# llm-d/llm-d-inference-scheduler

Measured on AMD Instinct MI355X. Metric: routed req/s + p50 EPP latency; P/D goodput (tok/s under TTFT SLO) Llama-3-8B, higher is better.
Workload: dtype bf16; 1 GPU; model=llama-3-8b, global_batch=256, seq_len=2048, parallelism=dp1, mode=mono, prompt_len=1024, kv_cache_dtype=bfloat16, warmup_steps_run=32, errors=0

## Files before the change

csrc/hip/hip_common.h:

```cpp
#pragma once
#include <hip/hip_runtime.h>
#include <hip/hip_bf16.h>
#include <cstdint>
#include <type_traits>

#define WAVE 64

typedef __attribute__((ext_vector_type(8))) short short8;
typedef __attribute__((ext_vector_type(4))) short short4v;
typedef __attribute__((ext_vector_type(4))) float float4v;
typedef __attribute__((ext_vector_type(2))) float float2v;

__device__ __forceinline__ float bf16_to_f32(short u) {
  union { float f; uint32_t i; } c;
  c.i = ((uint32_t)(uint16_t)u) << 16;
  return c.f;
}

__device__ __forceinline__ short f32_to_bf16(float f) {
  union { float f; uint32_t i; } c;
  c.f = f;
  uint32_t lsb = (c.i >> 16) & 1;
  uint32_t rounded = c.i + 0x7FFF + lsb;
  return (short)(uint16_t)(rounded >> 16);
}

typedef __attribute__((ext_vector_type(8))) unsigned char uchar8;

__device__ __forceinline__ void load_kv8(const short* p, float* f) {
  short8 v = *(const short8*)p;
#pragma unroll
  for (int j = 0; j < 8; ++j) f[j] = bf16_to_f32(v[j]);
}

__device__ __forceinline__ void load_kv8(const unsigned char* p, float* f) {
  const uint32_t* w = (const uint32_t*)p;
  uint32_t a = w[0], b = w[1];
  f[0] = __builtin_amdgcn_cvt_f32_fp8(a, 0);
  f[1] = __builtin_amdgcn_cvt_f32_fp8(a, 1);
  f[2] = __builtin_amdgcn_cvt_f32_fp8(a, 2);
  f[3] = __builtin_amdgcn_cvt_f32_fp8(a, 3);
  f[4] = __builtin_amdgcn_cvt_f32_fp8(b, 0);
  f[5] = __builtin_amdgcn_cvt_f32_fp8(b, 1);
  f[6] = __builtin_amdgcn_cvt_f32_fp8(b, 2);
  f[7] = __builtin_amdgcn_cvt_f32_fp8(b, 3);
}

__device__ __forceinline__ void load_kv2(const short* p, float& a, float& b) {
  const int32_t pair = *(const int32_t*)p;
  a = bf16_to_f32((short)(pair & 0xFFFF));
  b = bf16_to_f32((short)((pair >> 16) & 0xFFFF));
}

__device__ __forceinline__ void load_kv2(const unsigned char* p, float& a,
                                         float& b) {
  const uint32_t pair = *(const uint16_t*)p;
  a = __builtin_amdgcn_cvt_f32_fp8(pair, 0);
// ... 102 lines not shown
```

csrc/hip/launchers.h:

```cpp
#pragma once
#include <hip/hip_runtime.h>
#include <cstdint>


hipError_t lds_hash_prompts(const int32_t* tokens, const int64_t* offsets,
                            int n_requests, int block_tokens, int max_blocks,
                            uint64_t seed0, uint64_t* out, int32_t* counts,
                            hipStream_t stream);
hipError_t lds_table_update(uint64_t* keys, unsigned long long* masks,
                            uint32_t cap_mask, const uint64_t* hashes,
                            int64_t n, int endpoint, int is_remove,
                            unsigned int* dropped, hipStream_t stream);
hipError_t lds_match_longest(const uint64_t* keys,
                             const unsigned long long* masks,
                             uint32_t cap_mask, const uint64_t* hashes,
                             const int32_t* counts, int n_requests,
                             int max_blocks, int n_endpoints, int32_t* out,
                             hipStream_t stream);


hipError_t lds_rmsnorm(const void* x, void* residual, const void* w, void* y,
                       int64_t n_rows, int H, float eps, hipStream_t stream);
hipError_t lds_rope(void* q, void* k, const float* cos_sin,
                    const int32_t* positions, int n_tokens, int n_q_heads,
                    int n_kv_heads, int head_dim, hipStream_t stream);
hipError_t lds_silu_mul(const void* gate_up, void* y, int64_t T, int I,
                        hipStream_t stream);


hipError_t lds_reshape_and_cache(const void* k_new, const void* v_new,
                                 void* k_cache, void* v_cache,
                                 const int64_t* slots, int n_tokens, int kvh,
                                 int bs, int d, int kv_fp8,
                                 const float* k_inv_scale,
                                 const float* v_inv_scale,
                                 hipStream_t stream);
hipError_t lds_gather_blocks(const void* pool, void* staging,
                             const int32_t* block_ids, int n_sel, int n_layers,
                             int64_t n_blocks, int64_t block_bytes,
                             int is_scatter, hipStream_t stream);
hipError_t lds_copy_blocks_peer(const void* src_pool, void* dst_pool,
                                const int32_t* src_ids, const int32_t* dst_ids,
                                int n_sel, int n_layers, int64_t src_nb,
                                int64_t dst_nb, int64_t block_bytes,
                                hipStream_t stream);


constexpr int FLASH_GLDS_BT_CAP = 1024;

struct AttnArgs {
  const void* q;
  const void* k_cache;
  const void* v_cache;
  const int32_t* block_tables;
  void* out;
  const float* k_scale;
  const float* v_scale;
  int n_q_heads, kvh, bs, head_dim, max_blocks;
  int kv_fp8;
  float scale;
// ... 56 lines not shown
```

csrc/hip/norm_rope_act.hip:

```cpp
#include "hip_common.h"
#include "launchers.h"

namespace {

constexpr int RMSNORM_WAVES = 4;

template <bool RESIDUAL>
__global__ void rmsnorm_kernel(const short* __restrict__ x,
                               short* __restrict__ residual,
                               const short* __restrict__ w,
                               short* __restrict__ y, int H, float eps) {
  constexpr int CACHE_CHUNKS = 8;
  __shared__ float red[16];
  const int64_t row = blockIdx.x;
  const int tid = threadIdx.x;
  const int nthreads = blockDim.x;
  const short8* x8 = (const short8*)(x + row * H);
  short8* r8 = RESIDUAL ? (short8*)(residual + row * H) : nullptr;
  const short8* w8 = (const short8*)w;
  short8* y8 = (short8*)(y + row * H);
  const int nchunks = H / 8;

  float vals[CACHE_CHUNKS][8];
  float ss = 0.f;
// ... 25 lines not shown
  ci = 0;
  for (int c = tid; c < nchunks; c += nthreads, ++ci) {
    float f[8];
    if (ci < CACHE_CHUNKS) {
#pragma unroll
      for (int j = 0; j < 8; ++j) f[j] = vals[ci][j];
    } else {
      short8 v = RESIDUAL ? r8[c] : x8[c];
#pragma unroll
      for (int j = 0; j < 8; ++j) f[j] = bf16_to_f32(v[j]);
    }
    short8 wv = w8[c];
    short8 o;
#pragma unroll
    for (int j = 0; j < 8; ++j) o[j] = f32_to_bf16(f[j] * inv * bf16_to_f32(wv[j]));
    y8[c] = o;
  }
}

__global__ void rope_kernel(short* __restrict__ q, short* __restrict__ k,
                            const float* __restrict__ cos_sin,
                            const int32_t* __restrict__ positions, int n_tokens,
                            int n_q_heads, int n_kv_heads, int D) {
  const int t = blockIdx.x;
  const int head = blockIdx.y;
  const int half = D / 2;
  const int lane = threadIdx.x;
  if (t >= n_tokens || lane >= half) return;
  short* base = (head < n_q_heads)
                    ? q + ((int64_t)t * n_q_heads + head) * D
                    : k + ((int64_t)t * n_kv_heads + (head - n_q_heads)) * D;
  const float* cs = cos_sin + ((int64_t)positions[t] * half + lane) * 2;
  const float c = cs[0], s = cs[1];
  float x1 = bf16_to_f32(base[lane]);
  float x2 = bf16_to_f32(base[lane + half]);
  base[lane] = f32_to_bf16(x1 * c - x2 * s);
  base[lane + half] = f32_to_bf16(x2 * c + x1 * s);
}

__global__ void silu_mul_kernel(const short* __restrict__ gate_up,
                                short* __restrict__ y, int64_t T, int I) {
  const int nchunks = I / 8;
  const int64_t total = T * nchunks;
  for (int64_t i = (int64_t)blockIdx.x * blockDim.x + threadIdx.x; i < total;
       i += (int64_t)gridDim.x * blockDim.x) {
    int64_t row = i / nchunks;
    int c = (int)(i % nchunks);
    const short8* g8 = (const short8*)(gate_up + row * 2 * I);
    const short8* u8 = (const short8*)(gate_up + row * 2 * I + I);
    short8 g = g8[c], u = u8[c];
    short8 o;
#pragma unroll
    for (int j = 0; j < 8; ++j) {
      float gf = bf16_to_f32(g[j]);
      float uf = bf16_to_f32(u[j]);
      float sig = 1.f / (1.f + __expf(-gf));
      o[j] = f32_to_bf16(gf * sig * uf);
    }
    ((short8*)(y + row * I))[c] = o;
  }
}

}

hipError_t lds_rmsnorm(const void* x, void* residual, const void* w, void* y,
                       int64_t n_rows, int H, float eps, hipStream_t stream) {
  if (n_rows == 0) return hipSuccess;
  dim3 grid((uint32_t)n_rows), block(RMSNORM_WAVES * WAVE);
  if (residual) {
    hipLaunchKernelGGL(rmsnorm_kernel<true>, grid, block, 0, stream,
// ... 37 lines not shown
```

csrc/hip/ops.hip:

```cpp
#include <torch/extension.h>
#include <ATen/hip/HIPContext.h>
#include <ATen/hip/impl/HIPStreamMasqueradingAsCUDA.h>

#include <hip/hip_runtime.h>

#include <climits>

#include "launchers.h"

#define CHECK_HIP(expr)                                                    \
  do {                                                                     \
    hipError_t err__ = (expr);                                             \
    TORCH_CHECK(err__ == hipSuccess, "HIP error: ", hipGetErrorString(err__)); \
  } while (0)

#define CHECK_GPU(t) TORCH_CHECK((t).is_cuda() && (t).is_contiguous(), #t " must be contiguous on GPU")

namespace {

int kv_fp8_flag(const torch::Tensor& cache) {
  if (cache.scalar_type() == at::kFloat8_e4m3fn) return 1;
  TORCH_CHECK(cache.scalar_type() == at::kBFloat16,
              "KV cache must be bf16 or fp8_e4m3fn");
  return 0;
// ... 204 lines not shown
  auto y = torch::empty(sizes, gate_up.options());
  CHECK_HIP(lds_silu_mul(gate_up.data_ptr(), y.data_ptr(), T, I,
                         cur_stream()));
  return y;
}

void reshape_and_cache(torch::Tensor k_new, torch::Tensor v_new,
                       torch::Tensor k_cache, torch::Tensor v_cache,
                       torch::Tensor slots,
                       c10::optional<torch::Tensor> k_inv_scale,
                       c10::optional<torch::Tensor> v_inv_scale) {
  check_tensor(k_new, "k_new", k_new, "k_new", at::kBFloat16,
               {ANY, ANY, ANY});
  const int64_t T = k_new.size(0), KVH = k_new.size(1), D = k_new.size(2);
  TORCH_CHECK(D % 8 == 0, "head dim k_new.size(2) must be a multiple of 8, "
              "got ", D);
  check_int(KVH * (D / 8), 1, INT_MAX, "KVH * D / 8");
  check_tensor(v_new, "v_new", k_new, "k_new", at::kBFloat16, {T, KVH, D});
  const int fp8 = kv_fp8_flag(k_cache);
  check_tensor(k_cache, "k_cache", k_new, "k_new", k_cache.scalar_type(),
               {ANY, KVH, ANY, D});
  check_tensor(v_cache, "v_cache", k_new, "k_new", k_cache.scalar_type(),
               k_cache.sizes());
  const int bs = check_int(k_cache.size(2), 1, INT_MAX,
                           "block size k_cache.size(2)");
  check_tensor(slots, "slots", k_new, "k_new", at::kLong, {T});
  const float* kis = kv_scale_ptr(k_inv_scale, k_cache, "k_inv_scale");
  const float* vis = kv_scale_ptr(v_inv_scale, v_cache, "v_inv_scale");
  CHECK_HIP(lds_reshape_and_cache(
      k_new.data_ptr(), v_new.data_ptr(), k_cache.data_ptr(),
      v_cache.data_ptr(), slots.data_ptr<int64_t>(),
      check_int(T, 0, INT_MAX, "k_new.size(0)"), (int)KVH, bs, (int)D, fp8,
      kis, vis, cur_stream()));
}

int64_t check_pool(const torch::Tensor& pool, const char* name) {
  check_tensor(pool, name, pool, name, pool.scalar_type(),
               {ANY, 2, ANY, ANY, ANY, ANY});
  TORCH_CHECK(pool.size(0) <= INT_MAX, name, " has too many layers (",
              pool.size(0), ")");
  const int64_t block_bytes = pool.size(3) * pool.size(4) * pool.size(5) *
                              (int64_t)pool.element_size();
  TORCH_CHECK(block_bytes % 16 == 0, name, ": one block (", block_bytes,
              " bytes) must be a multiple of 16 bytes");
  return block_bytes;
}

void move_blocks(torch::Tensor pool, torch::Tensor staging,
                 torch::Tensor block_ids, bool is_scatter) {
  const int64_t block_bytes = check_pool(pool, "pool");
  check_tensor(block_ids, "block_ids", pool, "pool", at::kInt, {ANY});
  const int64_t n = block_ids.size(0);
  check_tensor(staging, "staging", pool, "pool", pool.scalar_type(),
               {n, pool.size(0), 2, pool.size(3), pool.size(4), pool.size(5)});
  CHECK_HIP(lds_gather_blocks(pool.data_ptr(), staging.data_ptr(),
                              block_ids.data_ptr<int32_t>(),
                              check_int(n, 0, INT_MAX, "block_ids.size(0)"),
                              (int)pool.size(0), pool.size(2), block_bytes,
                              is_scatter ? 1 : 0, cur_stream()));
}


torch::Tensor ipc_alloc_tensor(std::vector<int64_t> shape,
                               torch::Tensor like) {
  int64_t numel = 1;
  for (auto s : shape) numel *= s;
// ... 61 lines not shown
  check_tensor(k_cache, "k_cache", q, "q", k_cache.scalar_type(),
               {ANY, ANY, ANY, 128});
  check_tensor(v_cache, "v_cache", q, "q", k_cache.scalar_type(),
               k_cache.sizes());
  a.kvh = check_int(k_cache.size(1), 1, GRID_YZ_MAX, "KV heads");
  a.bs = check_int(k_cache.size(2), 1, INT_MAX, "block size k_cache.size(2)");
  const int64_t QH = q.size(1), qpg = QH / a.kvh;
  TORCH_CHECK(QH % a.kvh == 0 &&
              (qpg == 1 || qpg == 2 || qpg == 4 || qpg == 8),
              "q heads (", QH, ") must be 1, 2, 4 or 8 times the KV heads (",
              a.kvh, ")");
  a.n_q_heads = (int)QH;
  a.head_dim = 128;
  check_tensor(block_tables, "block_tables", q, "q", at::kInt, {ANY, ANY});
  a.max_blocks = check_int(block_tables.size(1), 1, INT_MAX,
                           "max_blocks = block_tables.size(1)");
  a.k_scale = kv_scale_ptr(k_scale, k_cache, "k_scale");
  a.v_scale = kv_scale_ptr(v_scale, v_cache, "v_scale");
  a.q = q.data_ptr();
  a.k_cache = k_cache.data_ptr();
  a.v_cache = v_cache.data_ptr();
  a.block_tables = block_tables.data_ptr<int32_t>();
  a.scale = (float)scale;
  return a;
}

AttnArgs check_decode(const torch::Tensor& q, const torch::Tensor& k_cache,
                      const torch::Tensor& v_cache,
                      const torch::Tensor& block_tables,
                      const torch::Tensor& seq_lens, double scale,
                      int64_t chunk,
                      const c10::optional<torch::Tensor>& k_scale,
                      const c10::optional<torch::Tensor>& v_scale) {
  AttnArgs a = check_attention(q, k_cache, v_cache, block_tables, scale,
                               k_scale, v_scale);
  const int64_t B = block_tables.size(0);
  TORCH_CHECK(q.size(0) == B, "q (", q.size(0), " rows) and block_tables (",
              B, " rows) must hold one row per sequence");
  check_tensor(seq_lens, "seq_lens", q, "q", at::kInt, {B});
  TORCH_CHECK(chunk == 256 || chunk == 512, "chunk must be 256 or 512, got ",
              chunk);
  a.seq_lens = seq_lens.data_ptr<int32_t>();
  a.n_seqs = (int)B;
  a.chunk = (int)chunk;
  return a;
}

torch::Tensor paged_attention(torch::Tensor q, torch::Tensor k_cache,
                              torch::Tensor v_cache,
                              torch::Tensor block_tables,
                              torch::Tensor seq_lens, double scale,
                              int64_t chunk,
                              c10::optional<torch::Tensor> k_scale,
                              c10::optional<torch::Tensor> v_scale) {
  AttnArgs a = check_decode(q, k_cache, v_cache, block_tables, seq_lens,
                            scale, chunk, k_scale, v_scale);
  auto out = torch::empty_like(q);
  a.out = out.data_ptr();
  CHECK_HIP(lds_paged_attention(a, cur_stream()));
  return out;
}

torch::Tensor paged_attention_split(torch::Tensor q, torch::Tensor k_cache,
                                    torch::Tensor v_cache,
                                    torch::Tensor block_tables,
                                    torch::Tensor seq_lens, int64_t n_parts,
// ... 188 lines not shown
              "rows, tokens, offsets and n_prompt must be contiguous");
  TORCH_CHECK(n_prompt.numel() == rows.numel() &&
              offsets.numel() == rows.numel() + 1,
              "n_prompt must hold one value per row and offsets one more, "
              "got ", rows.numel(), " rows, ", n_prompt.numel(),
              " n_prompt, ", offsets.numel(), " offsets");
  TORCH_CHECK(rows.numel() < (1LL << 31), "too many rows");
  CHECK_HIP(lds_token_state_fill(
      state.data_ptr<int16_t>(), (int)state.size(0), state.size(1), (int)V,
      rows.data_ptr<int32_t>(), (int)rows.numel(),
      tokens.data_ptr<int32_t>(), tokens.numel(),
      offsets.data_ptr<int64_t>(), n_prompt.data_ptr<int32_t>(),
      cur_stream()));
}

}

PYBIND11_MODULE(TORCH_EXTENSION_NAME, m) {
  m.doc() = "MI355X gfx950 kernels: prefix-cache hashing/match, paged KV, decode attention";
  m.def("hash_prompts", &hash_prompts, "batched chained block hashing");
  m.def("table_update", &table_update, "device prefix table insert/remove",
        py::arg("keys"), py::arg("masks"), py::arg("hashes"),
        py::arg("endpoint"), py::arg("is_remove"),
        py::arg("dropped") = py::none());
  m.def("match_longest", &match_longest, "device longest-prefix match");
  m.def("rmsnorm", &rmsnorm, py::arg("x"), py::arg("w"), py::arg("eps"),
        py::arg("residual") = py::none());
  m.def("rope", &rope, "in-place NeoX RoPE");
  m.def("silu_mul", &silu_mul, "fused SiLU*up on packed gate_up");
  m.def("reshape_and_cache", &reshape_and_cache,
        "scatter K/V into paged pool", py::arg("k_new"), py::arg("v_new"),
        py::arg("k_cache"), py::arg("v_cache"), py::arg("slots"),
        py::arg("k_inv_scale") = py::none(),
        py::arg("v_inv_scale") = py::none());
  m.def("move_blocks", &move_blocks, "gather/scatter KV blocks for xGMI transfer");
  m.def("ipc_alloc_tensor", &ipc_alloc_tensor,
        "hipMalloc-backed tensor (IPC-shareable, outside the caching allocator)");
  m.def("ipc_handle", &ipc_handle, "hipIpcGetMemHandle of a tensor");
  m.def("ipc_open", &ipc_open, "map a peer pool (hipIpcOpenMemHandle)");
  m.def("ipc_close", &ipc_close, "unmap a peer pool");
  m.def("copy_blocks_peer", &copy_blocks_peer,
        "one-sided xGMI pull of KV blocks from a mapped peer pool");
  m.def("paged_attention", &paged_attention,
        "GQA decode attention over paged KV", py::arg("q"),
        py::arg("k_cache"), py::arg("v_cache"), py::arg("block_tables"),
        py::arg("seq_lens"), py::arg("scale"), py::arg("chunk") = 256,
        py::arg("k_scale") = py::none(), py::arg("v_scale") = py::none());
  m.def("paged_attention_split", &paged_attention_split,
        "flash-decoding GQA attention with sequence partitioning",
        py::arg("q"), py::arg("k_cache"), py::arg("v_cache"),
        py::arg("block_tables"), py::arg("seq_lens"), py::arg("n_parts"),
        py::arg("part_tokens"), py::arg("scale"), py::arg("chunk") = 256,
        py::arg("k_scale") = py::none(), py::arg("v_scale") = py::none());
  m.def("flash_prefill", &flash_prefill,
        "fused MFMA causal varlen prefill attention over paged KV",
        py::arg("q"), py::arg("k_cache"), py::arg("v_cache"),
        py::arg("block_tables"), py::arg("seq_meta"), py::arg("tiles"),
        py::arg("scale"), py::arg("k_scale") = py::none(),
        py::arg("v_scale") = py::none());
  m.def("sample", &sample,
        "fused temperature/top-k/top-p/seeded sampler with logprobs -> "
        "(tokens, logprobs, n_kept, threshold)",
        py::arg("logits"), py::arg("temperature"), py::arg("top_k"),
        py::arg("top_p"), py::arg("seed"), py::arg("pos"));
  m.def("sample_ext", &sample_ext,
        "sample with penalties from the token state, min_p and top-N -> "
// ... 12 lines not shown
```

csrc/hip/paged_attention.hip:

```cpp
#include "hip_common.h"
#include "launchers.h"

namespace {

constexpr int D = 128;
constexpr int DEF_CHUNK = 256;
constexpr int NW = 4;
constexpr float NEG = -1e30f;

template <int QPG, bool SPLIT, typename CT, int CHUNK = DEF_CHUNK>
__global__ __launch_bounds__(NW * WAVE) void paged_attention_kernel(
    const short* __restrict__ q,
    const CT* __restrict__ k_cache,
    const CT* __restrict__ v_cache,
    const int32_t* __restrict__ block_tables,
    const int32_t* __restrict__ seq_lens,
    short* __restrict__ out,
    float* __restrict__ part_o,
    float* __restrict__ part_ml,
    const float* __restrict__ k_scale,
    const float* __restrict__ v_scale,
    int kvh, int bs, int max_blocks, int part_tokens, float scale) {
  const int b = blockIdx.x;
  const int kh = blockIdx.y;
  const int part = SPLIT ? blockIdx.z : 0;
  const int np = SPLIT ? gridDim.z : 1;
  const int qh0 = kh * QPG;
  const int n_q_heads = kvh * QPG;
  const int seq_len = seq_lens[b];
  const int t_begin = SPLIT ? part * part_tokens : 0;
  const int t_end = SPLIT ? min(seq_len, t_begin + part_tokens) : seq_len;

  __shared__ float q_lds[QPG][D];
  __shared__ float logits[QPG][CHUNK];
  __shared__ float m_sh[QPG], l_sh[QPG], alpha_sh[QPG];
  __shared__ float comb[NW][QPG][D];

  const int tid = threadIdx.x;
  const int wave = tid / WAVE;
  const int lane = tid % WAVE;

  if (SPLIT && t_begin >= seq_len) {
    if (tid < QPG) {
      float* ml = part_ml + ((((int64_t)b * kvh + kh) * np + part) * QPG +
                             tid) * 2;
      ml[0] = NEG;
      ml[1] = 0.f;
    }
    return;
  }

  const float q_scale = k_scale != nullptr ? scale * k_scale[kh] : scale;
  for (int i = tid; i < QPG * D; i += NW * WAVE) {
    int h = i / D, d = i % D;
    q_lds[h][d] =
        bf16_to_f32(q[((int64_t)b * n_q_heads + qh0 + h) * D + d]) * q_scale;
  }
  if (tid < QPG) {
    m_sh[tid] = NEG;
    l_sh[tid] = 0.f;
  }
  __syncthreads();

  float o_acc[QPG][2];
#pragma unroll
  for (int h = 0; h < QPG; ++h) o_acc[h][0] = o_acc[h][1] = 0.f;

  const int32_t* bt = block_tables + (int64_t)b * max_blocks;

  for (int chunk0 = t_begin; chunk0 < t_end; chunk0 += CHUNK) {
    const int n_t = min(CHUNK, t_end - chunk0);
    for (int tb = 0; tb < CHUNK; tb += NW * WAVE) {
      const int t_local = tb + wave * WAVE + lane;
      float dot[QPG];
#pragma unroll
      for (int h = 0; h < QPG; ++h) dot[h] = 0.f;
      if (t_local < n_t) {
        const int t = chunk0 + t_local;
        const int64_t blk = bt[t / bs];
        const int row = t % bs;
        const CT* krow = k_cache + (((blk * kvh + kh) * bs) + row) * D;
#pragma unroll 8
        for (int c = 0; c < D / 8; ++c) {
          float kf[8];
          load_kv8(krow + c * 8, kf);
#pragma unroll
          for (int h = 0; h < QPG; ++h) {
            const float4v* q4 = (const float4v*)&q_lds[h][c * 8];
            float4v qa = q4[0], qb = q4[1];
            dot[h] += qa[0] * kf[0] + qa[1] * kf[1] + qa[2] * kf[2] +
                      qa[3] * kf[3] + qb[0] * kf[4] + qb[1] * kf[5] +
                      qb[2] * kf[6] + qb[3] * kf[7];
          }
        }
      }
#pragma unroll
      for (int h = 0; h < QPG; ++h)
        logits[h][t_local] = (t_local < n_t) ? dot[h] : NEG;
    }
    __syncthreads();

    for (int h = wave; h < QPG; h += NW) {
      float lmax = NEG;
#pragma unroll
      for (int i = 0; i < CHUNK / WAVE; ++i)
        lmax = fmaxf(lmax, logits[h][i * WAVE + lane]);
      lmax = wave_reduce_max(lmax);
      const float m_old = m_sh[h];
      const float m_new = fmaxf(m_old, lmax);
      float lsum = 0.f;
#pragma unroll
      for (int i = 0; i < CHUNK / WAVE; ++i) {
        const int idx = i * WAVE + lane;
        float p = (logits[h][idx] <= NEG) ? 0.f : __expf(logits[h][idx] - m_new);
        logits[h][idx] = p;
        lsum += p;
      }
      lsum = wave_reduce_sum(lsum);
      if (lane == 0) {
        const float alpha = (m_old <= NEG) ? 0.f : __expf(m_old - m_new);
        alpha_sh[h] = alpha;
        l_sh[h] = l_sh[h] * alpha + lsum;
        m_sh[h] = m_new;
      }
    }
    __syncthreads();

#pragma unroll
    for (int h = 0; h < QPG; ++h) {
      const float a = alpha_sh[h];
      o_acc[h][0] *= a;
      o_acc[h][1] *= a;
    }
    {
      const int t_base = wave * (CHUNK / NW);
      const int t_cnt = min(CHUNK / NW, n_t - t_base);
      int i = 0;
      for (; i + 8 <= t_cnt; i += 8) {
        const CT* vrows[8];
#pragma unroll
        for (int j = 0; j < 8; ++j) {
          const int t = chunk0 + t_base + i + j;
          const int64_t blk = bt[t / bs];
          vrows[j] = v_cache + (((blk * kvh + kh) * bs) + t % bs) * D +
                     lane * 2;
        }
        float vv[8][2];
#pragma unroll
        for (int j = 0; j < 8; ++j) load_kv2(vrows[j], vv[j][0], vv[j][1]);
#pragma unroll
        for (int j = 0; j < 8; ++j) {
#pragma unroll
          for (int h = 0; h < QPG; ++h) {
            const float p = logits[h][t_base + i + j];
            o_acc[h][0] += p * vv[j][0];
            o_acc[h][1] += p * vv[j][1];
          }
        }
      }
      for (; i < t_cnt; ++i) {
        const int t = chunk0 + t_base + i;
        const int64_t blk = bt[t / bs];
        float v0, v1;
        load_kv2(v_cache + (((blk * kvh + kh) * bs) + t % bs) * D + lane * 2,
                 v0, v1);
#pragma unroll
        for (int h = 0; h < QPG; ++h) {
          const float p = logits[h][t_base + i];
          o_acc[h][0] += p * v0;
          o_acc[h][1] += p * v1;
        }
      }
    }
    __syncthreads();
  }

  if (v_scale != nullptr) {
    const float vs = v_scale[kh];
#pragma unroll
    for (int h = 0; h < QPG; ++h) {
      o_acc[h][0] *= vs;
      o_acc[h][1] *= vs;
    }
  }

#pragma unroll
  for (int h = 0; h < QPG; ++h) {
    comb[wave][h][2 * lane] = o_acc[h][0];
    comb[wave][h][2 * lane + 1] = o_acc[h][1];
  }
  __syncthreads();
  if (SPLIT) {
    float* po = part_o + ((((int64_t)b * kvh + kh) * np + part) * QPG) * D;
    for (int i = tid; i < QPG * D; i += NW * WAVE) {
      const int h = i / D, d = i % D;
      float s = 0.f;
#pragma unroll
      for (int w = 0; w < NW; ++w) s += comb[w][h][d];
// ... 120 lines not shown
```

llm_d_inference_scheduler_amd/models/llama.py:

```python
import math
import os
from dataclasses import dataclass
from typing import Dict, List, Optional

import torch

from .. import ops
from ..ops import ref as ops_ref
from ..utils.logging import get_logger
from .configs import ModelConfig

log = get_logger("models.llama")

_TUNED_GEMM_LOADED = False


def _load_tuned_gemms() -> None:
    global _TUNED_GEMM_LOADED
    if _TUNED_GEMM_LOADED:
        return
    _TUNED_GEMM_LOADED = True
    path = os.path.join(os.path.dirname(os.path.abspath(__file__)),
                        "..", "..", "profiles", "tuned_gemm_gfx950.csv")
    if os.environ.get("LLMD_NO_TUNED_GEMM", "0") == "1":
# ... 3 lines not shown
        tunable.enable(True)
        tunable.tuning_enable(False)
        tunable.read_file(path)
        log.info("loaded tuned GEMM solutions", path=path)


@dataclass
class ForwardBatch:
    input_ids: torch.Tensor
    positions: torch.Tensor
    slot_mapping: torch.Tensor
    is_decode: bool
    block_tables: Optional[torch.Tensor] = None
    seq_lens: Optional[torch.Tensor] = None
    max_seq_len: Optional[int] = None
    seq_starts: Optional[List[int]] = None
    ctx_lens: Optional[List[int]] = None
    prefill_block_tables: Optional[List[torch.Tensor]] = None
    prefill_bt: Optional[torch.Tensor] = None
    prefill_meta: Optional[torch.Tensor] = None
    prefill_tiles: Optional[torch.Tensor] = None
    logit_rows: Optional[torch.Tensor] = None
    embed_rows: Optional[torch.Tensor] = None
    embed_values: Optional[torch.Tensor] = None


class LlamaRunner:
    def __init__(self, config: ModelConfig, device: torch.device,
                 dtype: torch.dtype = torch.bfloat16, seed: int = 0):
        self.cfg = config
        self.device = device
        self.dtype = dtype
        self.scale = 1.0 / math.sqrt(config.head_dim)
        c = config
        if self.device.type == "cuda":
            _load_tuned_gemms()
            torch.cuda.manual_seed_all(seed)

            def w(*shape, std=0.02):
                t = torch.empty(*shape, dtype=torch.float32,
                                device=self.device)
                t.normal_(0.0, std)
                return t.to(dtype)
        else:
            gen = torch.Generator(device="cpu").manual_seed(seed)

            def w(*shape, std=0.02):
                t = torch.empty(*shape, dtype=torch.float32)
                t.normal_(0.0, std, generator=gen)
                return t.to(dtype).to(device)

        out_std = 0.02 / math.sqrt(2 * c.num_layers)
        self.embed = w(c.vocab_size, c.hidden_size)
        self.layers: List[Dict[str, torch.Tensor]] = []
        for _ in range(c.num_layers):
            self.layers.append({
                "input_norm": torch.ones(c.hidden_size, dtype=dtype,
                                         device=device),
                "wqkv": w(c.hidden_size, c.q_size + 2 * c.kv_size),
                "wo": w(c.q_size, c.hidden_size, std=out_std),
                "post_norm": torch.ones(c.hidden_size, dtype=dtype,
                                        device=device),
                **({"q_norm": torch.ones(c.head_dim, dtype=dtype,
                                         device=device),
                    "k_norm": torch.ones(c.head_dim, dtype=dtype,
                                         device=device)}
                   if c.qk_norm else {}),
                "wgate_up": w(c.hidden_size, 2 * c.intermediate_size),
                "wdown": w(c.intermediate_size, c.hidden_size, std=out_std),
            })
        self.final_norm = torch.ones(c.hidden_size, dtype=dtype, device=device)
        self.lm_head = self.embed if c.tie_embeddings else \
            w(c.vocab_size, c.hidden_size)
        self.cos_sin = ops_ref.rope_table(c.max_position, c.head_dim,
                                          c.rope_theta, device=device)

    def weight_bytes(self) -> int:
        total = self.embed.numel() + self.lm_head.numel() + \
            self.final_norm.numel()
        for layer in self.layers:
            total += sum(t.numel() for t in layer.values())
        return total * self.embed.element_size()

    def forward(self, batch: ForwardBatch, kv_pool: torch.Tensor,
                embeddings_out: bool = False,
                kv_scales=None, kv_observer=None) -> torch.Tensor:
        c = self.cfg
        hidden = self.embed[batch.input_ids]
        if batch.embed_rows is not None and batch.embed_rows.numel():
            hidden[batch.embed_rows] = batch.embed_values.to(hidden.dtype)
        residual = None
        pos32 = batch.positions.to(torch.int32)
        for li, layer in enumerate(self.layers):
            if residual is None:
                residual = hidden.clone()
                normed = ops.rmsnorm(hidden, layer["input_norm"], c.rms_eps)
            else:
                normed = ops.rmsnorm(hidden, layer["input_norm"], c.rms_eps,
                                     residual=residual)
            qkv = normed @ layer["wqkv"]
            q, k, v = qkv.split([c.q_size, c.kv_size, c.kv_size], dim=-1)
            T = q.shape[0]
            q = q.view(T, c.num_heads, c.head_dim).contiguous()
            k = k.view(T, c.num_kv_heads, c.head_dim).contiguous()
            v = v.view(T, c.num_kv_heads, c.head_dim).contiguous()
            if c.qk_norm:
                q = ops.rmsnorm(q.view(T * c.num_heads, c.head_dim),
                                layer["q_norm"],
                                c.rms_eps).view(T, c.num_heads, c.head_dim)
                k = ops.rmsnorm(k.view(T * c.num_kv_heads, c.head_dim),
                                layer["k_norm"],
                                c.rms_eps).view(T, c.num_kv_heads,
                                                c.head_dim)
            ops.rope(q, k, self.cos_sin, pos32)
            k_cache = kv_pool[li, 0]
            v_cache = kv_pool[li, 1]
            if kv_observer is not None:
                kv_observer(li, k, v)
            k_scale = v_scale = k_inv = v_inv = None
            if kv_scales is not None:
                k_scale, v_scale, k_inv, v_inv = kv_scales[li]
            ops.reshape_and_cache(k, v, k_cache, v_cache, batch.slot_mapping,
                                  k_inv_scale=k_inv, v_inv_scale=v_inv)
            if batch.is_decode:
                attn = ops.paged_attention(q, k_cache, v_cache,
                                           batch.block_tables, batch.seq_lens,
                                           self.scale,
                                           max_seq_len=batch.max_seq_len,
                                           k_scale=k_scale, v_scale=v_scale)
            else:
                attn = self._prefill_attention(batch, q, k_cache, v_cache,
                                               k_scale, v_scale)
            o = attn.view(T, c.q_size) @ layer["wo"]
            normed2 = ops.rmsnorm(o, layer["post_norm"], c.rms_eps,
                                  residual=residual)
            gate_up = normed2 @ layer["wgate_up"]
            act = ops.silu_mul(gate_up)
            hidden = act @ layer["wdown"]
        final = ops.rmsnorm(hidden, self.final_norm, c.rms_eps,
                            residual=residual)
        if embeddings_out:
            return final
        rows = batch.logit_rows
        sel = final if rows is None else final[rows]
        return sel @ self.lm_head.t()

    def _prefill_attention(self, batch: ForwardBatch, q: torch.Tensor,
                           k_cache: torch.Tensor,
                           v_cache: torch.Tensor,
                           k_scale: Optional[torch.Tensor] = None,
                           v_scale: Optional[torch.Tensor] = None
                           ) -> torch.Tensor:
        c = self.cfg
        if (q.is_cuda and batch.prefill_tiles is not None
                and c.head_dim == 128
                and c.num_heads // c.num_kv_heads in (1, 2, 4, 8)):
# ... 29 lines not shown
```

llm_d_inference_scheduler_amd/ops/__init__.py:

```python
from .dispatch import (
    flash_prefill, hip_ops, move_blocks, paged_attention, reshape_and_cache,
    rmsnorm, rope, sample, sample_ext, silu_mul, token_state_alloc,
    token_state_fill,
)
```

llm_d_inference_scheduler_amd/ops/dispatch.py:

```python
from typing import Optional

import torch

from . import ref

try:
    from .. import _hip_ops as _ext
except ImportError:
    _ext = None


def hip_ops():
    if _ext is None:
        raise RuntimeError(
            "_hip_ops extension is not built; run "
            "`python setup.py build_ext --inplace` (gfx950 HIP kernels are "
            "mandatory on GPU hosts — no eager fallback)")
    return _ext


def _use_hip(t: torch.Tensor) -> bool:
    if not t.is_cuda:
        return False
    hip_ops()
# ... 3 lines not shown
def rmsnorm(x: torch.Tensor, w: torch.Tensor, eps: float,
            residual: Optional[torch.Tensor] = None) -> torch.Tensor:
    if _use_hip(x):
        return _ext.rmsnorm(x, w, eps, residual)
    return ref.rmsnorm(x, w, eps, residual)


def rope(q: torch.Tensor, k: torch.Tensor, cos_sin: torch.Tensor,
         positions: torch.Tensor) -> None:
    if _use_hip(q):
        _ext.rope(q, k, cos_sin, positions.to(torch.int32))
        return
    ref.rope(q, k, cos_sin, positions)


def silu_mul(gate_up: torch.Tensor) -> torch.Tensor:
    if _use_hip(gate_up):
        return _ext.silu_mul(gate_up)
    return ref.silu_mul(gate_up)


def reshape_and_cache(k_new: torch.Tensor, v_new: torch.Tensor,
                      k_cache: torch.Tensor, v_cache: torch.Tensor,
                      slots: torch.Tensor, *,
                      k_inv_scale: Optional[torch.Tensor] = None,
                      v_inv_scale: Optional[torch.Tensor] = None) -> None:
    if _use_hip(k_new):
        _ext.reshape_and_cache(k_new, v_new, k_cache, v_cache,
                               slots.to(torch.int64), k_inv_scale,
                               v_inv_scale)
        return
    ref.reshape_and_cache(k_new, v_new, k_cache, v_cache, slots,
                          k_inv_scale=k_inv_scale, v_inv_scale=v_inv_scale)


import os as _os

_ATTN_CHUNK = int(_os.environ.get("LLMD_ATTN_CHUNK", "256"))


def split_geometry(n_wgs: int, max_seq_len: Optional[int],
                   chunk: int = _ATTN_CHUNK):
    if max_seq_len is None or n_wgs >= 1024 or max_seq_len <= 512:
        return None
    target_np = min(64, max(1, 1024 // max(1, n_wgs)))
    part = max(chunk, ((max_seq_len + target_np - 1) // target_np
                       + chunk - 1) // chunk * chunk)
    np_ = (max_seq_len + part - 1) // part
    return (np_, part) if np_ > 1 else None


def paged_attention(q: torch.Tensor, k_cache: torch.Tensor,
                    v_cache: torch.Tensor, block_tables: torch.Tensor,
                    seq_lens: torch.Tensor, scale: float,
                    max_seq_len: Optional[int] = None, *,
                    k_scale: Optional[torch.Tensor] = None,
                    v_scale: Optional[torch.Tensor] = None) -> torch.Tensor:
    if _use_hip(q):
        bt = block_tables.to(torch.int32)
        sl = seq_lens.to(torch.int32)
        geom = split_geometry(q.shape[0] * k_cache.shape[1], max_seq_len)
        if geom is not None:
            return _ext.paged_attention_split(q, k_cache, v_cache, bt, sl,
                                              geom[0], geom[1], scale,
                                              _ATTN_CHUNK, k_scale, v_scale)
        return _ext.paged_attention(q, k_cache, v_cache, bt, sl, scale,
# ... 62 lines not shown
```

setup.py:

```python
import os
import sys

from setuptools import setup

os.environ.setdefault("PYTORCH_ROCM_ARCH", "gfx950")

from pybind11.setup_helpers import Pybind11Extension
from torch.utils import cpp_extension

ROOT = os.path.dirname(os.path.abspath(__file__))

router_core = Pybind11Extension(
    "llm_d_inference_scheduler_amd._router_core",
    sources=["csrc/router/bindings.cpp"],
    cxx_std=17,
    extra_compile_args=["-O3"],
)

hip_ops = cpp_extension.CUDAExtension(
    name="llm_d_inference_scheduler_amd._hip_ops",
    sources=[
        "csrc/hip/ops.hip",
        "csrc/hip/prefix_kernels.hip",
        "csrc/hip/norm_rope_act.hip",
        "csrc/hip/kv_cache.hip",
        "csrc/hip/paged_attention.hip",
        "csrc/hip/flash_prefill.hip",
        "csrc/hip/flash_prefill_glds.hip",
        "csrc/hip/sampler.hip",
    ],
    extra_compile_args={
        "cxx": ["-O3"],
        "nvcc": ["-O3", "--offload-arch=gfx950", "-std=c++17"],
    },
)

ext_modules = [router_core]
if os.environ.get("LDS_AMD_SKIP_HIP", "0") != "1":
    ext_modules.append(hip_ops)

setup(
    name="llm_d_inference_scheduler_amd",
    version="0.1.0",
    packages=["llm_d_inference_scheduler_amd"],
    ext_modules=ext_modules,
    cmdclass={"build_ext": cpp_extension.BuildExtension.with_options(use_ninja=True)},
)
```

Measured before the change: 12680 tok/s.

## Fuse QKV split, RoPE and KV-cache write into one epilogue kernel

Adds a kernel that reads the QKV GEMM output once, rotates Q and K with RoPE, writes Q to a fresh tensor and scatters rotated K and V into the paged cache. This replaces three contiguous copies, a RoPE launch and a reshape_and_cache launch per layer. Paged attention now stores each K row's pool index in shared memory so the V pass reuses it instead of recomputing block-table lookups, and the QPG==8 variant gets a waves-per-EU occupancy hint. The fused path only runs for bf16 KV without qk_norm or an observer. It computes RoPE with FMA, so low-order rounding may differ slightly from the old kernel.

```diff
diff --git a/csrc/hip/hip_common.h b/csrc/hip/hip_common.h
--- a/csrc/hip/hip_common.h
+++ b/csrc/hip/hip_common.h
@@ -23,6 +23,15 @@
   uint32_t lsb = (c.i >> 16) & 1;
   uint32_t rounded = c.i + 0x7FFF + lsb;
   return (short)(uint16_t)(rounded >> 16);
+}
+
+__device__ __forceinline__ void rope_rotate_pair(short x1_bf16, short x2_bf16,
+                                                 float c, float s, short& o1,
+                                                 short& o2) {
+  const float x1 = bf16_to_f32(x1_bf16);
+  const float x2 = bf16_to_f32(x2_bf16);
+  o1 = f32_to_bf16(__builtin_fmaf(x1, c, -(x2 * s)));
+  o2 = f32_to_bf16(__builtin_fmaf(x1, s, x2 * c));
 }
 
 typedef __attribute__((ext_vector_type(8))) unsigned char uchar8;
diff --git a/csrc/hip/launchers.h b/csrc/hip/launchers.h
--- a/csrc/hip/launchers.h
+++ b/csrc/hip/launchers.h
@@ -26,6 +26,14 @@
                     int n_kv_heads, int head_dim, hipStream_t stream);
 hipError_t lds_silu_mul(const void* gate_up, void* y, int64_t T, int I,
                         hipStream_t stream);
+
+
+hipError_t lds_qkv_rope_cache(const void* qkv, const float* cos_sin,
+                              const int32_t* positions, const int64_t* slots,
+                              void* q_out, void* k_cache, void* v_cache,
+                              int64_t n_tokens, int n_q_heads, int kvh, int bs,
+                              int d, int kv_fp8, const float* k_inv_scale,
+                              const float* v_inv_scale, hipStream_t stream);
 
 
 hipError_t lds_reshape_and_cache(const void* k_new, const void* v_new,
diff --git a/csrc/hip/norm_rope_act.hip b/csrc/hip/norm_rope_act.hip
--- a/csrc/hip/norm_rope_act.hip
+++ b/csrc/hip/norm_rope_act.hip
@@ -81,10 +81,10 @@
                     : k + ((int64_t)t * n_kv_heads + (head - n_q_heads)) * D;
   const float* cs = cos_sin + ((int64_t)positions[t] * half + lane) * 2;
   const float c = cs[0], s = cs[1];
-  float x1 = bf16_to_f32(base[lane]);
-  float x2 = bf16_to_f32(base[lane + half]);
-  base[lane] = f32_to_bf16(x1 * c - x2 * s);
-  base[lane + half] = f32_to_bf16(x2 * c + x1 * s);
+  short o1, o2;
+  rope_rotate_pair(base[lane], base[lane + half], c, s, o1, o2);
+  base[lane] = o1;
+  base[lane + half] = o2;
 }
 
 __global__ void silu_mul_kernel(const short* __restrict__ gate_up,
diff --git a/csrc/hip/ops.hip b/csrc/hip/ops.hip
--- a/csrc/hip/ops.hip
+++ b/csrc/hip/ops.hip
@@ -260,6 +260,53 @@
       v_cache.data_ptr(), slots.data_ptr<int64_t>(),
       check_int(T, 0, INT_MAX, "k_new.size(0)"), (int)KVH, bs, (int)D, fp8,
       kis, vis, cur_stream()));
+}
+
+void check_aligned16(const torch::Tensor& t, const char* name) {
+  TORCH_CHECK(((uintptr_t)t.data_ptr() & 15u) == 0, name,
+              " must be 16-byte aligned");
+}
+
+torch::Tensor qkv_rope_cache(torch::Tensor qkv, torch::Tensor cos_sin,
+                             torch::Tensor positions, torch::Tensor slots,
+                             torch::Tensor k_cache, torch::Tensor v_cache,
+                             int64_t n_q_heads,
+                             c10::optional<torch::Tensor> k_inv_scale,
+                             c10::optional<torch::Tensor> v_inv_scale) {
+  check_tensor(qkv, "qkv", qkv, "qkv", at::kBFloat16, {ANY, ANY});
+  const int64_t T = check_int(qkv.size(0), 0, INT_MAX, "qkv.size(0)");
+  const int fp8 = kv_fp8_flag(k_cache);
+  check_tensor(k_cache, "k_cache", qkv, "qkv", k_cache.scalar_type(),
+               {ANY, ANY, ANY, ANY});
+  check_tensor(v_cache, "v_cache", qkv, "qkv", k_cache.scalar_type(),
+               k_cache.sizes());
+  const int kvh = check_int(k_cache.size(1), 1, 65536, "KV heads");
+  const int bs = check_int(k_cache.size(2), 1, INT_MAX,
+                           "block size k_cache.size(2)");
+  const int64_t D = k_cache.size(3);
+  TORCH_CHECK(D % 16 == 0, "head dim k_cache.size(3) must be a multiple of "
+              "16, got ", D);
+  const int d = check_int(D, 16, 2048, "head dim k_cache.size(3)");
+  const int qh = check_int(n_q_heads, 1, 65536, "n_q_heads");
+  TORCH_CHECK(qkv.size(1) == (qh + 2 * (int64_t)kvh) * D, "qkv.size(1) must "
+              "be (n_q_heads + 2 * KV heads) * head dim = ",
+              (qh + 2 * (int64_t)kvh) * D, ", got ", qkv.size(1));
+  check_tensor(cos_sin, "cos_sin", qkv, "qkv", at::kFloat, {ANY, D / 2, 2});
+  check_tensor(positions, "positions", qkv, "qkv", at::kInt, {T});
+  check_tensor(slots, "slot_mapping", qkv, "qkv", at::kLong, {T});
+  const float* kis = kv_scale_ptr(k_inv_scale, k_cache, "k_inv_scale");
+  const float* vis = kv_scale_ptr(v_inv_scale, v_cache, "v_inv_scale");
+  check_aligned16(qkv, "qkv");
+  check_aligned16(cos_sin, "cos_sin");
+  check_aligned16(k_cache, "k_cache");
+  check_aligned16(v_cache, "v_cache");
+  auto q = torch::empty({T, qh, D}, qkv.options());
+  CHECK_HIP(lds_qkv_rope_cache(
+      qkv.data_ptr(), cos_sin.data_ptr<float>(),
+      positions.data_ptr<int32_t>(), slots.data_ptr<int64_t>(), q.data_ptr(),
+      k_cache.data_ptr(), v_cache.data_ptr(), T, qh, kvh, bs, d, fp8, kis,
+      vis, cur_stream()));
+  return q;
 }
 
 int64_t check_pool(const torch::Tensor& pool, const char* name) {
@@ -387,6 +434,12 @@
                       int64_t chunk,
                       const c10::optional<torch::Tensor>& k_scale,
                       const c10::optional<torch::Tensor>& v_scale) {
+  if (k_cache.dim() == 4) {
+    const int64_t pool_rows =
+        k_cache.size(0) * k_cache.size(1) * k_cache.size(2);
+    TORCH_CHECK(pool_rows < (int64_t(1) << 31), "KV cache rows NB*KVH*BS (",
+                pool_rows, ") must be below 2^31");
+  }
   AttnArgs a = check_attention(q, k_cache, v_cache, block_tables, scale,
                                k_scale, v_scale);
   const int64_t B = block_tables.size(0);
@@ -641,6 +694,12 @@
         "scatter K/V into paged pool", py::arg("k_new"), py::arg("v_new"),
         py::arg("k_cache"), py::arg("v_cache"), py::arg("slots"),
         py::arg("k_inv_scale") = py::none(),
+        py::arg("v_inv_scale") = py::none());
+  m.def("qkv_rope_cache", &qkv_rope_cache,
+        "QKV GEMM epilogue: rotated q out, rotated K and V into the pool",
+        py::arg("qkv"), py::arg("cos_sin"), py::arg("positions"),
+        py::arg("slot_mapping"), py::arg("k_cache"), py::arg("v_cache"),
+        py::arg("n_q_heads"), py::arg("k_inv_scale") = py::none(),
         py::arg("v_inv_scale") = py::none());
   m.def("move_blocks", &move_blocks, "gather/scatter KV blocks for xGMI transfer");
   m.def("ipc_alloc_tensor", &ipc_alloc_tensor,
diff --git a/csrc/hip/paged_attention.hip b/csrc/hip/paged_attention.hip
--- a/csrc/hip/paged_attention.hip
+++ b/csrc/hip/paged_attention.hip
@@ -6,10 +6,13 @@
 constexpr int D = 128;
 constexpr int DEF_CHUNK = 256;
 constexpr int NW = 4;
+constexpr int V_BATCH = 8;
 constexpr float NEG = -1e30f;
 
 template <int QPG, bool SPLIT, typename CT, int CHUNK = DEF_CHUNK>
-__global__ __launch_bounds__(NW * WAVE) void paged_attention_kernel(
+__global__ __launch_bounds__(NW * WAVE)
+__attribute__((amdgpu_waves_per_eu(QPG == 8 ? 3 : 1))) void
+paged_attention_kernel(
     const short* __restrict__ q,
     const CT* __restrict__ k_cache,
     const CT* __restrict__ v_cache,
@@ -35,6 +38,7 @@
   __shared__ float logits[QPG][CHUNK];
   __shared__ float m_sh[QPG], l_sh[QPG], alpha_sh[QPG];
   __shared__ float comb[NW][QPG][D];
+  __shared__ __attribute__((aligned(16))) int32_t row_idx[CHUNK];
 
   const int tid = threadIdx.x;
   const int wave = tid / WAVE;
@@ -79,7 +83,9 @@
         const int t = chunk0 + t_local;
         const int64_t blk = bt[t / bs];
         const int row = t % bs;
-        const CT* krow = k_cache + (((blk * kvh + kh) * bs) + row) * D;
+        const int64_t pool_row = ((blk * kvh + kh) * bs) + row;
+        row_idx[t_local] = (int32_t)pool_row;
+        const CT* krow = k_cache + pool_row * D;
 #pragma unroll 8
         for (int c = 0; c < D / 8; ++c) {
           float kf[8];
@@ -135,21 +141,19 @@
     {
       const int t_base = wave * (CHUNK / NW);
       const int t_cnt = min(CHUNK / NW, n_t - t_base);
+      const CT* v_lane = v_cache + lane * 2;
       int i = 0;
-      for (; i + 8 <= t_cnt; i += 8) {
-        const CT* vrows[8];
-#pragma unroll
-        for (int j = 0; j < 8; ++j) {
-          const int t = chunk0 + t_base + i + j;
-          const int64_t blk = bt[t / bs];
-          vrows[j] = v_cache + (((blk * kvh + kh) * bs) + t % bs) * D +
-                     lane * 2;
-        }
-        float vv[8][2];
-#pragma unroll
-        for (int j = 0; j < 8; ++j) load_kv2(vrows[j], vv[j][0], vv[j][1]);
-#pragma unroll
-        for (int j = 0; j < 8; ++j) {
+      for (; i + V_BATCH <= t_cnt; i += V_BATCH) {
+        const CT* vrows[V_BATCH];
+#pragma unroll
+        for (int j = 0; j < V_BATCH; ++j)
+          vrows[j] = v_lane + (int64_t)row_idx[t_base + i + j] * D;
+        float vv[V_BATCH][2];
+#pragma unroll
+        for (int j = 0; j < V_BATCH; ++j)
+          load_kv2(vrows[j], vv[j][0], vv[j][1]);
+#pragma unroll
+        for (int j = 0; j < V_BATCH; ++j) {
 #pragma unroll
           for (int h = 0; h < QPG; ++h) {
             const float p = logits[h][t_base + i + j];
@@ -159,11 +163,8 @@
         }
       }
       for (; i < t_cnt; ++i) {
-        const int t = chunk0 + t_base + i;
-        const int64_t blk = bt[t / bs];
         float v0, v1;
-        load_kv2(v_cache + (((blk * kvh + kh) * bs) + t % bs) * D + lane * 2,
-                 v0, v1);
+        load_kv2(v_lane + (int64_t)row_idx[t_base + i] * D, v0, v1);
 #pragma unroll
         for (int h = 0; h < QPG; ++h) {
           const float p = logits[h][t_base + i];
diff --git a/csrc/hip/qkv_epilogue.hip b/csrc/hip/qkv_epilogue.hip
--- /dev/null
+++ b/csrc/hip/qkv_epilogue.hip
@@ -0,0 +1,113 @@
+#include "hip_common.h"
+#include "launchers.h"
+
+namespace {
+
+__device__ __forceinline__ void rope_rotate8(short8& lo, short8& hi,
+                                             const float* __restrict__ cs) {
+  const float4v* cs4 = (const float4v*)cs;
+  float4v t[4] = {cs4[0], cs4[1], cs4[2], cs4[3]};
+#pragma unroll
+  for (int j = 0; j < 8; ++j) {
+    const float c = t[j / 2][(j % 2) * 2];
+    const float s = t[j / 2][(j % 2) * 2 + 1];
+    short o1, o2;
+    rope_rotate_pair(lo[j], hi[j], c, s, o1, o2);
+    lo[j] = o1;
+    hi[j] = o2;
+  }
+}
+
+template <typename CT>
+__device__ __forceinline__ void store_kv8_scaled(CT* p, short8 v,
+                                                 const float* inv_scale,
+                                                 int h) {
+  if constexpr (std::is_same<CT, unsigned char>::value) {
+    if (inv_scale != nullptr) {
+      store_kv8(p, v, inv_scale[h]);
+      return;
+    }
+  }
+  store_kv8(p, v);
+}
+
+template <typename CT>
+__global__ __launch_bounds__(256) void qkv_rope_cache_kernel(
+    const short* __restrict__ qkv, const float* __restrict__ cos_sin,
+    const int32_t* __restrict__ positions, const int64_t* __restrict__ slots,
+    short* __restrict__ q_out, CT* __restrict__ k_cache,
+    CT* __restrict__ v_cache, const float* __restrict__ k_inv_scale,
+    const float* __restrict__ v_inv_scale, int64_t n_tokens, int qh, int kvh,
+    int bs, int d) {
+  const int half = d / 2;
+  const int lanes = d / 16;
+  const int heads = qh + 2 * kvh;
+  const int64_t total = n_tokens * heads * lanes;
+  for (int64_t i = (int64_t)blockIdx.x * blockDim.x + threadIdx.x; i < total;
+       i += (int64_t)gridDim.x * blockDim.x) {
+    const int d0 = (int)(i % lanes) * 8;
+    const int64_t task = i / lanes;
+    const int head = (int)(task % heads);
+    const int64_t t = task / heads;
+    const short* src = qkv + (t * heads + head) * d + d0;
+    if (head < qh) {
+      short8 lo = *(const short8*)src;
+      short8 hi = *(const short8*)(src + half);
+      rope_rotate8(lo, hi,
+                   cos_sin + ((int64_t)positions[t] * half + d0) * 2);
+      short* dst = q_out + (t * qh + head) * d + d0;
+      *(short8*)dst = lo;
+      *(short8*)(dst + half) = hi;
+      continue;
+    }
+    const int64_t slot = slots[t];
+    if (slot < 0) continue;
+    short8 lo = *(const short8*)src;
+    short8 hi = *(const short8*)(src + half);
+    const bool is_k = head < qh + kvh;
+    const int h = is_k ? head - qh : head - qh - kvh;
+    const int64_t block = slot / bs, row = slot % bs;
+    const int64_t dst_off = (((block * kvh + h) * bs) + row) * d + d0;
+    if (is_k) {
+      rope_rotate8(lo, hi,
+                   cos_sin + ((int64_t)positions[t] * half + d0) * 2);
+      store_kv8_scaled(k_cache + dst_off, lo, k_inv_scale, h);
+      store_kv8_scaled(k_cache + dst_off + half, hi, k_inv_scale, h);
+    } else {
+      store_kv8_scaled(v_cache + dst_off, lo, v_inv_scale, h);
+      store_kv8_scaled(v_cache + dst_off + half, hi, v_inv_scale, h);
+    }
+  }
+}
+
+}
+
+hipError_t lds_qkv_rope_cache(const void* qkv, const float* cos_sin,
+                              const int32_t* positions, const int64_t* slots,
+                              void* q_out, void* k_cache, void* v_cache,
+                              int64_t n_tokens, int n_q_heads, int kvh, int bs,
+                              int d, int kv_fp8, const float* k_inv_scale,
+                              const float* v_inv_scale, hipStream_t stream) {
+  if (n_tokens == 0) return hipSuccess;
+  const int threads = 256;
+  const int64_t total = n_tokens * (n_q_heads + 2 * kvh) * (d / 16);
+  int64_t blocks = (total + threads - 1) / threads;
+  if (blocks > 2048) blocks = 2048;
+  if (kv_fp8) {
+    hipLaunchKernelGGL(qkv_rope_cache_kernel<unsigned char>,
+                       dim3((uint32_t)blocks), dim3(threads), 0, stream,
+                       (const short*)qkv, cos_sin, positions, slots,
+                       (short*)q_out, (unsigned char*)k_cache,
+                       (unsigned char*)v_cache, k_inv_scale, v_inv_scale,
+                       n_tokens, n_q_heads, kvh, bs, d);
+  } else {
+    if (k_inv_scale || v_inv_scale) return hipErrorInvalidValue;
+    hipLaunchKernelGGL(qkv_rope_cache_kernel<short>, dim3((uint32_t)blocks),
+                       dim3(threads), 0, stream, (const short*)qkv, cos_sin,
+                       positions, slots, (short*)q_out, (short*)k_cache,
+                       (short*)v_cache, nullptr, nullptr, n_tokens, n_q_heads,
+                       kvh, bs, d);
+  }
+  HIP_CHECK_LAST();
+  return hipSuccess;
+}
diff --git a/llm_d_inference_scheduler_amd/models/llama.py b/llm_d_inference_scheduler_amd/models/llama.py
--- a/llm_d_inference_scheduler_amd/models/llama.py
+++ b/llm_d_inference_scheduler_amd/models/llama.py
@@ -59,6 +59,7 @@
         self.device = device
         self.dtype = dtype
         self.scale = 1.0 / math.sqrt(config.head_dim)
+        self._fused_qkv = True
         c = config
         if self.device.type == "cuda":
             _load_tuned_gemms()
@@ -118,6 +119,9 @@
             hidden[batch.embed_rows] = batch.embed_values.to(hidden.dtype)
         residual = None
         pos32 = batch.positions.to(torch.int32)
+        fused_qkv = (self._fused_qkv and kv_observer is None
+                     and kv_pool.dtype == torch.bfloat16
+                     and not c.qk_norm and c.head_dim % 16 == 0)
         for li, layer in enumerate(self.layers):
             if residual is None:
                 residual = hidden.clone()
@@ -126,29 +130,37 @@
                 normed = ops.rmsnorm(hidden, layer["input_norm"], c.rms_eps,
                                      residual=residual)
             qkv = normed @ layer["wqkv"]
-            q, k, v = qkv.split([c.q_size, c.kv_size, c.kv_size], dim=-1)
-            T = q.shape[0]
-            q = q.view(T, c.num_heads, c.head_dim).contiguous()
-            k = k.view(T, c.num_kv_heads, c.head_dim).contiguous()
-            v = v.view(T, c.num_kv_heads, c.head_dim).contiguous()
-            if c.qk_norm:
-                q = ops.rmsnorm(q.view(T * c.num_heads, c.head_dim),
-                                layer["q_norm"],
-                                c.rms_eps).view(T, c.num_heads, c.head_dim)
-                k = ops.rmsnorm(k.view(T * c.num_kv_heads, c.head_dim),
-                                layer["k_norm"],
-                                c.rms_eps).view(T, c.num_kv_heads,
-                                                c.head_dim)
-            ops.rope(q, k, self.cos_sin, pos32)
+            T = qkv.shape[0]
             k_cache = kv_pool[li, 0]
             v_cache = kv_pool[li, 1]
-            if kv_observer is not None:
-                kv_observer(li, k, v)
             k_scale = v_scale = k_inv = v_inv = None
             if kv_scales is not None:
                 k_scale, v_scale, k_inv, v_inv = kv_scales[li]
-            ops.reshape_and_cache(k, v, k_cache, v_cache, batch.slot_mapping,
-                                  k_inv_scale=k_inv, v_inv_scale=v_inv)
+            if fused_qkv:
+                q = ops.qkv_rope_cache(qkv, self.cos_sin, pos32,
+                                       batch.slot_mapping, k_cache, v_cache,
+                                       c.num_heads, k_inv_scale=k_inv,
+                                       v_inv_scale=v_inv)
+            else:
+                q, k, v = qkv.split([c.q_size, c.kv_size, c.kv_size], dim=-1)
+                q = q.view(T, c.num_heads, c.head_dim).contiguous()
+                k = k.view(T, c.num_kv_heads, c.head_dim).contiguous()
+                v = v.view(T, c.num_kv_heads, c.head_dim).contiguous()
+                if c.qk_norm:
+                    q = ops.rmsnorm(q.view(T * c.num_heads, c.head_dim),
+                                    layer["q_norm"],
+                                    c.rms_eps).view(T, c.num_heads,
+                                                    c.head_dim)
+                    k = ops.rmsnorm(k.view(T * c.num_kv_heads, c.head_dim),
+                                    layer["k_norm"],
+                                    c.rms_eps).view(T, c.num_kv_heads,
+                                                    c.head_dim)
+                ops.rope(q, k, self.cos_sin, pos32)
+                if kv_observer is not None:
+                    kv_observer(li, k, v)
+                ops.reshape_and_cache(k, v, k_cache, v_cache,
+                                      batch.slot_mapping,
+                                      k_inv_scale=k_inv, v_inv_scale=v_inv)
             if batch.is_decode:
                 attn = ops.paged_attention(q, k_cache, v_cache,
                                            batch.block_tables, batch.seq_lens,
diff --git a/llm_d_inference_scheduler_amd/ops/__init__.py b/llm_d_inference_scheduler_amd/ops/__init__.py
--- a/llm_d_inference_scheduler_amd/ops/__init__.py
+++ b/llm_d_inference_scheduler_amd/ops/__init__.py
@@ -1,5 +1,5 @@
 from .dispatch import (
-    flash_prefill, hip_ops, move_blocks, paged_attention, reshape_and_cache,
-    rmsnorm, rope, sample, sample_ext, silu_mul, token_state_alloc,
-    token_state_fill,
+    flash_prefill, hip_ops, move_blocks, paged_attention, qkv_rope_cache,
+    reshape_and_cache, rmsnorm, rope, sample, sample_ext, silu_mul,
+    token_state_alloc, token_state_fill,
 )
diff --git a/llm_d_inference_scheduler_amd/ops/dispatch.py b/llm_d_inference_scheduler_amd/ops/dispatch.py
--- a/llm_d_inference_scheduler_amd/ops/dispatch.py
+++ b/llm_d_inference_scheduler_amd/ops/dispatch.py
@@ -59,6 +59,30 @@
         return
     ref.reshape_and_cache(k_new, v_new, k_cache, v_cache, slots,
                           k_inv_scale=k_inv_scale, v_inv_scale=v_inv_scale)
+
+
+def qkv_rope_cache(qkv: torch.Tensor, cos_sin: torch.Tensor,
+                   positions: torch.Tensor, slot_mapping: torch.Tensor,
+                   k_cache: torch.Tensor, v_cache: torch.Tensor,
+                   n_q_heads: int, *,
+                   k_inv_scale: Optional[torch.Tensor] = None,
+                   v_inv_scale: Optional[torch.Tensor] = None
+                   ) -> torch.Tensor:
+    if _use_hip(qkv):
+        return _ext.qkv_rope_cache(qkv, cos_sin, positions.to(torch.int32),
+                                   slot_mapping.to(torch.int64), k_cache,
+                                   v_cache, n_q_heads, k_inv_scale,
+                                   v_inv_scale)
+    T = qkv.shape[0]
+    kvh, d = k_cache.shape[1], k_cache.shape[3]
+    q, k, v = qkv.split([n_q_heads * d, kvh * d, kvh * d], dim=-1)
+    q = q.reshape(T, n_q_heads, d).clone()
+    k = k.reshape(T, kvh, d).clone()
+    v = v.reshape(T, kvh, d)
+    ref.rope(q, k, cos_sin, positions)
+    ref.reshape_and_cache(k, v, k_cache, v_cache, slot_mapping,
+                          k_inv_scale=k_inv_scale, v_inv_scale=v_inv_scale)
+    return q
 
 
 import os as _os
diff --git a/setup.py b/setup.py
--- a/setup.py
+++ b/setup.py
@@ -23,6 +23,7 @@
         "csrc/hip/ops.hip",
         "csrc/hip/prefix_kernels.hip",
         "csrc/hip/norm_rope_act.hip",
+        "csrc/hip/qkv_epilogue.hip",
         "csrc/hip/kv_cache.hip",
         "csrc/hip/paged_attention.hip",
         "csrc/hip/flash_prefill.hip",
```

After: 14210 tok/s, median of 6. 1.12x the previous value.
